# naver/dust3r

Measured on NVIDIA H100. Metric: image-pairs/sec (512x384, ViT-L/B+DPT), higher is better.
Workload: dtype bf16

## Files before the change

dust3r_b200/_lib_fwd.py:

```python
import ctypes as C

F_BIAS, F_GELU, F_RELU, F_OUT_F32, F_RESID_INPLACE = 1, 2, 4, 8, 16
F_ADD0, F_ADD1, F_OUT2_RELU, F_ROPE, F_OUT2_BF16 = 32, 64, 128, 256, 2048


class Linear(C.Structure):
    _fields_ = [('w', C.c_void_p), ('b', C.c_void_p)]


class Norm(C.Structure):
    _fields_ = [('g', C.c_void_p), ('b', C.c_void_p)]


class EncBlock(C.Structure):
    _fields_ = [('norm1', Norm), ('norm2', Norm), ('qkv', Linear), ('proj', Linear), ('fc1', Linear), ('fc2', Linear)]


class DecBlock(C.Structure):
    _fields_ = [('norm1', Norm), ('norm2', Norm), ('norm3', Norm), ('norm_y', Norm),
                ('qkv', Linear), ('proj', Linear), ('projq', Linear), ('projkv', Linear), ('cproj', Linear),
                ('fc1', Linear), ('fc2', Linear)]


class Fusion(C.Structure):
# ... 27 lines not shown
    lib.d3r_conv3x3_bf16.argtypes = [vp, vp, vp, vp, vp, vp, vp, i32, i32, i32, i32, i32, u32, vp]
    lib.d3r_attention_hd64.restype = C.c_int
    lib.d3r_attention_hd64.argtypes = [vp, i64, vp, i64, vp, i64, vp, i64, i32, i32, i32, i32, f32, vp]
    lib.d3r_conv_transpose_bf16.restype = C.c_int
    lib.d3r_conv_transpose_bf16.argtypes = [vp, vp, vp, vp, i32, i32, i32, i32, i32, i32, vp]
    lib.d3r_conv3x3_head_tail.restype = C.c_int
    lib.d3r_conv3x3_head_tail.argtypes = [vp, vp, vp, vp, vp, vp, vp, i32, i32, i32, i32, i32, f32, f32, vp]
    lib.d3r_layernorm_bf16.restype = C.c_int
    lib.d3r_layernorm_bf16.argtypes = [vp, vp, vp, vp, i32, i32, f32, vp]
    lib.d3r_upsample2x_bf16.restype = C.c_int
    lib.d3r_upsample2x_bf16.argtypes = [vp, vp, i32, i32, i32, i32, i32, i32, vp]
    lib.d3r_im2col_3x3_s2_bf16.restype = C.c_int
    lib.d3r_im2col_3x3_s2_bf16.argtypes = [vp, vp, i32, i32, i32, i32, vp]
    lib.d3r_patch_im2col16.restype = C.c_int
    lib.d3r_patch_im2col16.argtypes = [vp, vp, i32, i32, i32, vp]
    lib.d3r_linear_head_postprocess.restype = C.c_int
    lib.d3r_linear_head_postprocess.argtypes = [vp, vp, vp, i32, i32, i32, i32, i32, i32, f32, f32, vp]
    lib.d3r_set_gemm_impl.restype = None
    lib.d3r_set_gemm_impl.argtypes = [i32]
    lib.d3r_set_gemm_store.restype = None
    lib.d3r_set_gemm_store.argtypes = [i32]
    lib.d3r_set_conv_store.restype = None
    lib.d3r_set_conv_store.argtypes = [i32]
    lib.d3r_set_attention_impl.restype = None
    lib.d3r_set_attention_impl.argtypes = [i32]
    lib.d3r_forward_workspace_bytes.restype = i64
    lib.d3r_forward_workspace_bytes.argtypes = [C.POINTER(Model), i32, i32, i32, i32]
    lib.d3r_forward_pairs.restype = C.c_int
    lib.d3r_forward_pairs.argtypes = [C.POINTER(Model), vp, i32, C.POINTER(i32), C.POINTER(i32), i32, i32, i32,
                                      vp, vp, vp, vp, vp, i64, vp]
    lib.d3r_forward_mixed_workspace_bytes.restype = i64
    lib.d3r_forward_mixed_workspace_bytes.argtypes = [C.POINTER(Model), i32, i32, i32, i32, i32]
    lib.d3r_forward_pairs_mixed.restype = C.c_int
    lib.d3r_forward_pairs_mixed.argtypes = [C.POINTER(Model), vp, i32, i32, vp, i32, i32, i32, vp, vp, vp, vp, vp, i64, vp]
    lib.d3r_encode_workspace_bytes.restype = i64
    lib.d3r_encode_workspace_bytes.argtypes = [C.POINTER(Model), i32, i32, i32]
    lib.d3r_encode_images.restype = C.c_int
    lib.d3r_encode_images.argtypes = [C.POINTER(Model), vp, i32, i32, i32, vp, vp, i64, vp]
    lib.d3r_decode_workspace_bytes.restype = i64
    lib.d3r_decode_workspace_bytes.argtypes = [C.POINTER(Model), i32, i32, i32, i32, i32]
    lib.d3r_decode_pairs.restype = C.c_int
    lib.d3r_decode_pairs.argtypes = [C.POINTER(Model), vp, i32, i32, i32, vp, i32, i32, i32, C.POINTER(i32), C.POINTER(i32), i32,
                                     vp, vp, vp, vp, vp, i64, vp]
    lib.d3r_forward_set_debug.restype = C.c_int
    lib.d3r_forward_set_debug.argtypes = [i32, vp, i64]
    lib.d3r_sizeof_model.restype = C.c_int
# ... 1 lines not shown
```

dust3r_b200/csrc/gemm_host.cu:

```cuda
#include "gemm_wgmma.cuh"
#include "gemm_host.h"
#include "prof.h"

namespace d3r {
namespace gemm {

static int pick_block_n(int N, int mode, uint32_t flags, int conv_m_tiles = 0) {
  if (flags & F_HEAD_FINAL) return 128;
  if (conv_m_tiles > 0) return (N == 256 && (conv_m_tiles + 1) / 2 >= 4 * (num_sms() / 2)) ? 256 : 128;
  if (N % 256 == 0 && pick_epi(mode, flags) != EPI_GENERIC) return 256;
  if (N % 128 == 0) return 128;
  if (N % 64 == 0) return 64;
  return (N > 128) ? 128 : 64;
}

static int g_impl = 2;
static int g_pair_min_kb = 4;
static bool use_pair(int bn, int num_kb) { return bn >= 128 && (g_impl == 1 || (g_impl == 2 && num_kb >= g_pair_min_kb)); }

static int g_store = 1;
static int g_conv_store = 1;

static int grid_for(bool pair, int m_tiles, int n_tiles) {
  if (pair) {
    const int items = ((m_tiles + 1) / 2) * n_tiles;
    const int max_clusters = num_sms() / 2;
    return 2 * (items < max_clusters ? items : max_clusters);
  }
  const int items = m_tiles * n_tiles;
  return items < num_sms() ? items : num_sms();
}

static const char* prof_tag(const Params& p, int bn, bool pair) {
  return (p.mode == 1) ? ((p.flags & F_HEAD_FINAL) ? (pair ? "conv3x3_head_tail_2cta" : "conv3x3_head_tail")
                                                   : (pair ? "conv3x3_wgmma_2cta" : "conv3x3_wgmma"))
                       : (bn == 256 ? (pair ? "gemm_wgmma_2cta_bn256" : "gemm_wgmma_bn256")
                                    : (pair ? "gemm_wgmma_2cta_bn128" : (bn == 128 ? "gemm_wgmma_bn128" : "gemm_wgmma_bn64")));
}

template <int BN, int EPI, bool PAIR, bool TMA_STORE = false>
static int launch(const CUtensorMap& ta, const CUtensorMap& tb, const CUtensorMap& to, const Params& p, int m_tiles, int n_tiles,
                  cudaStream_t st) {
  constexpr int kSmem = Cfg<BN, TMA_STORE>::kSmemBytes;
  static unsigned long long attr_devices = 0;
  if (first_launch_on_this_device(attr_devices))
    D3R_CUDA(cudaFuncSetAttribute(gemm_kernel<BN, EPI, PAIR, TMA_STORE>, cudaFuncAttributeMaxDynamicSharedMemorySize, kSmem));
  const int grid = grid_for(PAIR, m_tiles, n_tiles);
  char detail[96];
  snprintf(detail, sizeof(detail), "M=%d N=%d K=%d flags=0x%x mode=%d epi=%d", p.M, p.N, p.K, (unsigned)p.flags, p.mode, EPI);
  prof::Scope scope(prof_tag(p, BN, PAIR), st, 2.0 * double(p.M) * double(p.N) * double(p.K), 0.0, 1, detail);
  D3R_CUDA(pdl::launch_clustered(gemm_kernel<BN, EPI, PAIR, TMA_STORE>, dim3(grid), dim3(kNumThreads), size_t(kSmem), st, PAIR ? 2 : 1,
                                 ta, tb, to, p));
  D3R_LAUNCH_CHECK();
  return D3R_OK;
}

template <int BN, bool PAIR>
static int launch_conv(const CUtensorMap& ta, const CUtensorMap& tb, const CUtensorMap& to, const ConvMaps& cm, const Params& p,
                       int m_tiles, int n_tiles, cudaStream_t st) {
  constexpr int kSmem = Cfg<BN, true>::kSmemBytes;
  static unsigned long long attr_devices = 0;
  if (first_launch_on_this_device(attr_devices))
    D3R_CUDA(cudaFuncSetAttribute(conv_kernel<BN, PAIR>, cudaFuncAttributeMaxDynamicSharedMemorySize, kSmem));
  const int grid = grid_for(PAIR, m_tiles, n_tiles);
  char detail[96];
  snprintf(detail, sizeof(detail), "M=%d N=%d K=%d flags=0x%x mode=%d epi=%d", p.M, p.N, p.K, (unsigned)p.flags, p.mode, EPI_GENERIC);
  prof::Scope scope(prof_tag(p, BN, PAIR), st, 2.0 * double(p.M) * double(p.N) * double(p.K), 0.0, 1, detail);
  D3R_CUDA(pdl::launch_clustered(conv_kernel<BN, PAIR>, dim3(grid), dim3(kNumThreads), size_t(kSmem), st, PAIR ? 2 : 1, ta, tb, to, cm, p));
  D3R_LAUNCH_CHECK();
  return D3R_OK;
}

template <int BN, bool PAIR>
static int dispatch_epi(int epi, const CUtensorMap& ta, const CUtensorMap& tb, const CUtensorMap* to, const Params& p, int m_tiles,
                        int n_tiles, cudaStream_t st) {
  if constexpr (BN == 256) {
    if (to) {
      switch (epi) {
        case EPI_RESID: return launch<BN, EPI_RESID, PAIR, true>(ta, tb, *to, p, m_tiles, n_tiles, st);
// ... 6 lines not shown
    case EPI_RESID: return launch<BN, EPI_RESID, PAIR>(ta, tb, tb, p, m_tiles, n_tiles, st);
    case EPI_ACT: return launch<BN, EPI_ACT, PAIR>(ta, tb, tb, p, m_tiles, n_tiles, st);
    case EPI_ROPE: return launch<BN, EPI_ROPE, PAIR>(ta, tb, tb, p, m_tiles, n_tiles, st);
  }
  if constexpr (BN == 128) return launch<128, EPI_GENERIC, PAIR>(ta, tb, tb, p, m_tiles, n_tiles, st);
  set_error("no BLOCK_N %d kernel for the generic epilogue", BN);
  return D3R_ERR_INVALID;
}

static int dispatch(int bn, const CUtensorMap& ta, const CUtensorMap& tb, const CUtensorMap* to, const Params& p, int m_tiles,
                    cudaStream_t st) {
  const int n_tiles = (p.N + bn - 1) / bn;
  const int epi = (bn >= 128) ? pick_epi(p.mode, p.flags) : EPI_GENERIC;
  const bool pair = use_pair(bn, p.num_kb);
  switch (bn) {
    case 256: return pair ? dispatch_epi<256, true>(epi, ta, tb, to, p, m_tiles, n_tiles, st) : dispatch_epi<256, false>(epi, ta, tb, to, p, m_tiles, n_tiles, st);
    case 128: return pair ? dispatch_epi<128, true>(epi, ta, tb, nullptr, p, m_tiles, n_tiles, st) : dispatch_epi<128, false>(epi, ta, tb, nullptr, p, m_tiles, n_tiles, st);
    case 64: return launch<64, EPI_GENERIC, false>(ta, tb, tb, p, m_tiles, n_tiles, st);
  }
  set_error("unsupported BLOCK_N %d", bn);
  return D3R_ERR_INVALID;
}

static int make_tmap_b(CUtensorMap* m, const void* B, int N, int taps, int Kc, int bn, int num_kb, const char* op) {
  cuuint64_t dims[3] = {(cuuint64_t)Kc, (cuuint64_t)taps, (cuuint64_t)N};
  cuuint64_t str[2] = {(cuuint64_t)Kc * 2, (cuuint64_t)taps * Kc * 2};
  cuuint32_t box[3] = {(cuuint32_t)BLOCK_K, 1, (cuuint32_t)(use_pair(bn, num_kb) ? bn / 2 : bn)};
  return encode_tensor_map(m, B, 3, dims, str, box, op);
}

int gemm_bf16(const void* A, long long lda, const void* B, Params p, cudaStream_t st) {
  D3R_CHECK_ARG(A && B, "gemm: null operand");
  D3R_CHECK_ARG(p.M > 0 && p.N > 0 && p.K > 0, "gemm: bad shape %d %d %d", p.M, p.N, p.K);
  D3R_CHECK_ARG(p.N % 32 == 0, "gemm: N=%d must be a multiple of 32", p.N);
  D3R_CHECK_ARG(p.K % 8 == 0 && lda % 8 == 0, "gemm: K=%d / lda=%lld must be multiples of 8 (16-byte TMA strides)", p.K, lda);
  D3R_CHECK_ARG((reinterpret_cast<uintptr_t>(A) & 15) == 0 && (reinterpret_cast<uintptr_t>(B) & 15) == 0, "gemm: operands must be 16-byte aligned");
  p.mode = 0;
  p.num_kb = (p.K + BLOCK_K - 1) / BLOCK_K;
  const int bn = pick_block_n(p.N, p.mode, p.flags);
  CUtensorMap ta, tb;
  {
    cuuint64_t dims[2] = {(cuuint64_t)p.K, (cuuint64_t)p.M};
    cuuint64_t str[1] = {(cuuint64_t)lda * 2};
    cuuint32_t box[2] = {(cuuint32_t)BLOCK_K, (cuuint32_t)BLOCK_M};
    int rc = encode_tensor_map(&ta, A, 2, dims, str, box, "gemm");
    if (rc) return rc;
  }
  int rc = make_tmap_b(&tb, B, p.N, 1, p.K, bn, p.num_kb, "gemm");
  if (rc) return rc;
  CUtensorMap to;
  const bool f32 = (p.flags & F_RESID_INPLACE) != 0;
  const long long row_bytes = p.ldo * (f32 ? 4 : 2);
  const bool staged = g_store == 1 && bn == 256 && pick_epi(p.mode, p.flags) != EPI_GENERIC && p.ldo >= p.N && row_bytes % 16 == 0 &&
                      (reinterpret_cast<uintptr_t>(p.out) & 15) == 0;
  if (staged) {
    cuuint64_t dims[2] = {(cuuint64_t)p.N, (cuuint64_t)p.M};
    cuuint64_t str[1] = {(cuuint64_t)row_bytes};
    cuuint32_t box[2] = {(cuuint32_t)(f32 ? 32 : 64), 64};
    rc = encode_tensor_map(&to, p.out, 2, dims, str, box, "gemm output", f32 ? CU_TENSOR_MAP_DATA_TYPE_FLOAT32 : CU_TENSOR_MAP_DATA_TYPE_BFLOAT16);
    if (rc) return rc;
  }
  return dispatch(bn, ta, tb, staged ? &to : nullptr, p, (p.M + BLOCK_M - 1) / BLOCK_M, st);
}

static int make_tmap_conv_io(CUtensorMap* m, const void* base, int B, int H, int W, int C, int tile_w, const char* op) {
  const int bw = tile_w < 64 ? tile_w : 64;
  cuuint64_t dims[4] = {(cuuint64_t)C, (cuuint64_t)W, (cuuint64_t)H, (cuuint64_t)B};
  cuuint64_t str[3] = {(cuuint64_t)C * 2, (cuuint64_t)W * C * 2, (cuuint64_t)H * W * C * 2};
  cuuint32_t box[4] = {64, (cuuint32_t)bw, (cuuint32_t)(64 / bw), 1};
  return encode_tensor_map(m, base, 4, dims, str, box, op);
}

static bool aligned16(const void* ptr) { return (reinterpret_cast<uintptr_t>(ptr) & 15) == 0; }

int conv3x3_bf16(const void* x_nhwc, const void* w_packed, int B, int H, int W, int Cin, int Cout, Params p, cudaStream_t st) {
  D3R_CHECK_ARG(x_nhwc && w_packed, "conv3x3: null operand");
  D3R_CHECK_ARG(Cin % 8 == 0 && Cout % 32 == 0, "conv3x3: Cin=%d must be a multiple of 8 and Cout=%d of 32", Cin, Cout);
  p.mode = 1;
  p.M = B * H * W;
  p.N = Cout;
  p.cin_blocks = (Cin + BLOCK_K - 1) / BLOCK_K;
  p.K = 9 * Cin;
  p.num_kb = 9 * p.cin_blocks;
  p.cB = B; p.cH = H; p.cW = W;
  int tw = 16;
  while (tw < W && tw < 128) tw *= 2;
  p.tile_w = tw;
  p.tile_h = BLOCK_M / tw;
  p.tiles_x = (W + p.tile_w - 1) / p.tile_w;
  p.tiles_y = (H + p.tile_h - 1) / p.tile_h;
  p.ldo = Cout;
  const int m_tiles = B * p.tiles_x * p.tiles_y;
  const bool staged = g_conv_store == 1 && (Cout == 256 || Cout == 128) && (p.flags & ~EpiMask<EPI_CONV>::value) == 0 &&
                      aligned16(p.out) && (!(p.flags & F_OUT2_RELU) || aligned16(p.out2)) && (!(p.flags & F_ADD0) || aligned16(p.add0)) &&
                      (!(p.flags & F_ADD1) || aligned16(p.add1));
  const int bn = pick_block_n(p.N, p.mode, p.flags, staged ? m_tiles : 0);
  CUtensorMap ta, tb;
  {
    cuuint64_t dims[4] = {(cuuint64_t)Cin, (cuuint64_t)W, (cuuint64_t)H, (cuuint64_t)B};
    cuuint64_t str[3] = {(cuuint64_t)Cin * 2, (cuuint64_t)W * Cin * 2, (cuuint64_t)H * W * Cin * 2};
    cuuint32_t box[4] = {(cuuint32_t)BLOCK_K, (cuuint32_t)p.tile_w, (cuuint32_t)p.tile_h, 1};
    int rc = encode_tensor_map(&ta, x_nhwc, 4, dims, str, box, "conv3x3");
    if (rc) return rc;
  }
  int rc = make_tmap_b(&tb, w_packed, Cout, 9, Cin, bn, p.num_kb, "conv3x3");
  if (rc) return rc;
  if (!staged) return dispatch(bn, ta, tb, nullptr, p, m_tiles, st);
  CUtensorMap to;
  ConvMaps cm;
  rc = make_tmap_conv_io(&to, p.out, B, H, W, Cout, p.tile_w, "conv3x3 output");
  if (rc) return rc;
  cm.out2 = cm.add0 = cm.add1 = to;
  const struct { uint32_t flag; const void* base; CUtensorMap* map; const char* op; } io[3] = {
      {F_OUT2_RELU, p.out2, &cm.out2, "conv3x3 out2"}, {F_ADD0, p.add0, &cm.add0, "conv3x3 add0"}, {F_ADD1, p.add1, &cm.add1, "conv3x3 add1"}};
  for (const auto& t : io) {
    if (!(p.flags & t.flag)) continue;
    rc = make_tmap_conv_io(t.map, t.base, B, H, W, Cout, p.tile_w, t.op);
    if (rc) return rc;
  }
  const int n_tiles = Cout / bn;
  const bool pair = use_pair(bn, p.num_kb);
  if (bn == 256) return pair ? launch_conv<256, true>(ta, tb, to, cm, p, m_tiles, n_tiles, st) : launch_conv<256, false>(ta, tb, to, cm, p, m_tiles, n_tiles, st);
  return pair ? launch_conv<128, true>(ta, tb, to, cm, p, m_tiles, n_tiles, st) : launch_conv<128, false>(ta, tb, to, cm, p, m_tiles, n_tiles, st);
}

int conv_transpose_bf16(const void* x_nhwc, const void* w_packed, void* out, const float* bias, int B, int h, int w, int Cin, int Cout,
                        int k, cudaStream_t st) {
  D3R_CHECK_ARG(x_nhwc && w_packed && out, "conv_transpose: null buffer");
// ... 16 lines not shown
  D3R_CHECK_ARG(B > 0 && H > 0 && W > 0, "conv3x3_head_tail: bad shape B=%d H=%d W=%d", B, H, W);
  D3R_CHECK_ARG(depth_mode >= 0 && depth_mode <= 2, "conv3x3_head_tail: depth_mode %d out of range", depth_mode);
  D3R_CHECK_ARG(conf_mode >= 0 && conf_mode <= 2, "conv3x3_head_tail: conf_mode %d out of range", conf_mode);
  D3R_CHECK_ARG(conf_mode == 0 || conf, "conv3x3_head_tail: conf_mode %d without a conf buffer", conf_mode);
  Params p{};
  p.flags = F_HEAD_FINAL | (bias ? F_BIAS : 0);
  p.bias = bias;
  p.w4 = w4; p.b4 = b4;
  p.pts3d = pts3d; p.conf = conf;
  p.depth_mode = depth_mode; p.conf_mode = conf_mode;
  p.conf_min = conf_min; p.conf_max = conf_max;
  return conv3x3_bf16(x_nhwc, w_packed, B, H, W, 128, 128, p, st);
}

}
}

using namespace d3r;

extern "C" void d3r_set_gemm_impl(int32_t impl) { gemm::g_impl = impl; }
extern "C" void d3r_set_gemm_pair_min_kblocks(int32_t kb) { gemm::g_pair_min_kb = kb; }
extern "C" void d3r_set_gemm_store(int32_t store) { gemm::g_store = store; }
extern "C" void d3r_set_conv_store(int32_t store) { gemm::g_conv_store = store; }

extern "C" int d3r_gemm_bf16(const void* A, const void* B, void* out, const float* bias, const void* add0, void* out2,
                             int32_t M, int32_t N, int32_t K, int64_t ldo, uint32_t flags, const float* rope_cos,
                             const float* rope_sin, int32_t rope_cols, int32_t tokens_per_img, int32_t grid_w, void* stream) {
  gemm::Params p{};
  p.M = M; p.N = N; p.K = K;
  p.flags = flags;
  p.out = out; p.out2 = out2; p.add0 = add0; p.bias = bias; p.ldo = ldo;
  p.rope_cos = rope_cos; p.rope_sin = rope_sin; p.rope_cols = rope_cols; p.tokens_per_img = tokens_per_img; p.grid_w = grid_w;
  D3R_CHECK_ARG(!(flags & gemm::F_BIAS) || bias, "gemm: F_BIAS without bias");
  D3R_CHECK_ARG(!(flags & gemm::F_ROPE) || (rope_cos && rope_sin && tokens_per_img > 0 && grid_w > 0), "gemm: F_ROPE without tables");
  D3R_CHECK_ARG(!(flags & (gemm::F_CONVT | gemm::F_HEAD_FINAL)),
                "gemm: F_CONVT / F_HEAD_FINAL have their own entry points, d3r_conv_transpose_bf16 / d3r_conv3x3_head_tail");
  return gemm::gemm_bf16(A, K, B, p, (cudaStream_t)stream);
}

extern "C" int d3r_conv3x3_bf16(const void* x_nhwc, const void* w_packed, void* out, const float* bias, const void* add0,
                                const void* add1, void* out2, int32_t B, int32_t H, int32_t W, int32_t Cin, int32_t Cout,
                                uint32_t flags, void* stream) {
  gemm::Params p{};
  p.flags = flags;
  p.out = out; p.out2 = out2; p.add0 = add0; p.add1 = add1; p.bias = bias;
  D3R_CHECK_ARG(!(flags & (gemm::F_CONVT | gemm::F_HEAD_FINAL | gemm::F_ROPE)), "conv3x3: unsupported flag");
// ... 15 lines not shown
```

dust3r_b200/csrc/gemm_wgmma.cuh:

```cuda
#pragma once
#include "d3r_common.cuh"
#include "sm90_ptx.cuh"
#include "pdl.cuh"

namespace d3r {
namespace gemm {

constexpr int BLOCK_M = 128;
constexpr int BLOCK_K = 64;
constexpr int WGMMA_K = 16;
constexpr int kNumThreads = 384;
constexpr int kConsumerWarps = 8;

enum : uint32_t {
  F_BIAS = 1u << 0,
  F_GELU = 1u << 1,
  F_RELU = 1u << 2,
  F_OUT_F32 = 1u << 3,
  F_RESID_INPLACE = 1u << 4,
  F_ADD0 = 1u << 5,
  F_ADD1 = 1u << 6,
  F_OUT2_RELU = 1u << 7,
  F_ROPE = 1u << 8,
  F_CONVT = 1u << 9,
  F_HEAD_FINAL = 1u << 10,
  F_OUT2_BF16 = 1u << 11,
// ... 23 lines not shown
  int conf_mode;
  float conf_min, conf_max;
};

enum : int { EPI_GENERIC = 0, EPI_RESID = 1, EPI_ACT = 2, EPI_ROPE = 3, EPI_CONV = 4 };
template <int EPI> struct EpiMask { static constexpr uint32_t value = 0xFFFFFFFFu; };
template <> struct EpiMask<EPI_RESID> { static constexpr uint32_t value = F_BIAS | F_RESID_INPLACE; };
template <> struct EpiMask<EPI_ACT> { static constexpr uint32_t value = F_BIAS | F_GELU | F_RELU; };
template <> struct EpiMask<EPI_ROPE> { static constexpr uint32_t value = F_BIAS | F_ROPE; };
template <> struct EpiMask<EPI_CONV> { static constexpr uint32_t value = F_BIAS | F_RELU | F_ADD0 | F_ADD1 | F_OUT2_RELU; };

struct ConvMaps {
  CUtensorMap out2, add0, add1;
};

__host__ __device__ inline int pick_epi(int mode, uint32_t flags) {
  if (mode != 0) return EPI_GENERIC;
  if ((flags & ~F_BIAS) == F_RESID_INPLACE) return EPI_RESID;
  if ((flags & ~EpiMask<EPI_ACT>::value) == 0) return EPI_ACT;
  if ((flags & ~EpiMask<EPI_ROPE>::value) == 0) return EPI_ROPE;
  return EPI_GENERIC;
}

template <int BLOCK_N, bool TMA_STORE = false>
struct Cfg {
  static constexpr int kStageA = BLOCK_M * BLOCK_K * 2;
  static constexpr int kStageB = BLOCK_N * BLOCK_K * 2;
  static constexpr int kStages = (BLOCK_N == 256) ? 4 : (BLOCK_N == 128) ? 6 : 8;
  static constexpr int kRing = kStages * (kStageA + kStageB);
  static constexpr int kOutBuf = 64 * 128;
  static constexpr int kStaging = TMA_STORE ? 2 * 2 * kOutBuf : 0;
  static constexpr int kSmemBytes = kRing + kStaging + 1024  + 256  + (TMA_STORE ? 0 : (4 * 128 + 16) * 4) ;
  static_assert(kSmemBytes <= 227 * 1024, "shared memory of one CTA");
};

__device__ __forceinline__ float gelu_erf(float x) {
  constexpr float kU = 0.84932180028801904f;
  constexpr float kP = 0.3275911f * 0.70710678118654752f / kU;
  const float u = fabsf(x) * kU;
  const float t = ptx::rcp_approx(fmaf(kP, u, 1.f));
  float poly = fmaf(0.5f * 1.061405429f, t, 0.5f * -1.453152027f);
  poly = fmaf(poly, t, 0.5f * 1.421413741f);
  poly = fmaf(poly, t, 0.5f * -0.284496736f);
  poly = fmaf(poly, t, 0.5f * 0.254829592f);
  const float e = ptx::ex2_approx(-u * u);
  const float h = x * (poly * t * e);
  return fmaxf(x, 0.f) - fabsf(h);
}

template <int BLOCK_N, int EPI, bool PAIR, bool TMA_STORE>
__device__ __forceinline__ void gemm_body(const CUtensorMap& tmap_a, const CUtensorMap& tmap_b, const CUtensorMap& tmap_o,
                                          const ConvMaps* cm, const Params& p) {
  static_assert(EPI == EPI_CONV ? (TMA_STORE && (BLOCK_N == 256 || BLOCK_N == 128))
                                : (!TMA_STORE || (BLOCK_N == 256 && EPI != EPI_GENERIC)),
                "TMA-store epilogue: specialised projection epilogues on 128x256 tiles, the conv epilogue on 128x256 / 128x128");
  using C = Cfg<BLOCK_N, TMA_STORE>;
  extern __shared__ uint8_t smem_raw[];
  uint8_t* smem = reinterpret_cast<uint8_t*>((reinterpret_cast<uintptr_t>(smem_raw) + 1023) & ~uintptr_t(1023));
  uint8_t* smem_a = smem;
  uint8_t* smem_b = smem + C::kStages * C::kStageA;
  uint8_t* smem_o = smem + C::kRing;
  uint64_t* bars = reinterpret_cast<uint64_t*>(smem + C::kRing + C::kStaging);
  uint64_t* full_bar = bars;
  uint64_t* empty_bar = bars + C::kStages;
  uint64_t* add_bar = bars + 2 * C::kStages;
  float* s_w4 = reinterpret_cast<float*>(reinterpret_cast<uint8_t*>(bars) + 256);

  const int warp = threadIdx.x >> 5, lane = threadIdx.x & 31;
  const uint32_t rank = PAIR ? ptx::cluster_ctarank() : 0u;
  const int n_tiles = (p.N + BLOCK_N - 1) / BLOCK_N;
  const int m_tiles = (p.mode == 1) ? p.cB * p.tiles_y * p.tiles_x : (p.M + BLOCK_M - 1) / BLOCK_M;
  const int m_groups = PAIR ? (m_tiles + 1) / 2 : m_tiles;
  const int total_items = m_groups * n_tiles;
  const int first_item = PAIR ? blockIdx.x / 2 : blockIdx.x;
  const int item_stride = PAIR ? gridDim.x / 2 : gridDim.x;

  if (threadIdx.x == 0) {
    ptx::prefetch_tmap(&tmap_a);
    ptx::prefetch_tmap(&tmap_b);
    if constexpr (TMA_STORE) ptx::prefetch_tmap(&tmap_o);
    for (int s = 0; s < C::kStages; ++s) {
      ptx::mbar_init(ptx::smem_u32(&full_bar[s]), 1);
      ptx::mbar_init(ptx::smem_u32(&empty_bar[s]), (PAIR ? 2 : 1) * kConsumerWarps);
    }
    if constexpr (EPI == EPI_CONV) {
      ptx::prefetch_tmap(&cm->out2);
      ptx::prefetch_tmap(&cm->add0);
      ptx::prefetch_tmap(&cm->add1);
      ptx::mbar_init(ptx::smem_u32(&add_bar[0]), 1);
      ptx::mbar_init(ptx::smem_u32(&add_bar[1]), 1);
    }
    ptx::fence_barrier_init();
  }
  if (!TMA_STORE && (p.flags & F_HEAD_FINAL) && threadIdx.x >= 128) {
    for (int i = threadIdx.x - 128; i < 4 * 128 + 4; i += 256) s_w4[i] = (i < 512) ? p.w4[i] : p.b4[i - 512];
  }
  __syncthreads();
  if constexpr (PAIR) ptx::cluster_sync();
  pdl::sync_with_predecessor();

  if (warp < 4) {
    ptx::setmaxnreg_dec<40>();
    if (warp == 0 && ptx::elect_one()) {
      int stage = 0;
      uint32_t phase = 0;
      for (int item = first_item; item < total_items; item += item_stride) {
        const int tn = item % n_tiles, tm = (item / n_tiles) * (PAIR ? 2 : 1) + int(rank);
        int cb = 0, cy0 = 0, cx0 = 0;
        if (p.mode == 1) {
          cb = tm / (p.tiles_y * p.tiles_x);
          const int r = tm - cb * (p.tiles_y * p.tiles_x);
          cy0 = (r / p.tiles_x) * p.tile_h;
          cx0 = (r % p.tiles_x) * p.tile_w;
        }
        for (int kb = 0; kb < p.num_kb; ++kb) {
          ptx::mbar_wait(ptx::smem_u32(&empty_bar[stage]), phase ^ 1);
          const uint32_t fb = ptx::smem_u32(&full_bar[stage]);
          ptx::mbar_arrive_expect_tx(fb, C::kStageA + C::kStageB);
          const uint32_t sa = ptx::smem_u32(smem_a + stage * C::kStageA);
          const uint32_t sb = ptx::smem_u32(smem_b + stage * C::kStageB);
          int ka, kt = 0;
          if (p.mode == 1) {
            const int tap = kb / p.cin_blocks, cblk = kb - tap * p.cin_blocks;
            const int dy = tap / 3, dx = tap - dy * 3;
            ptx::tma_load_4d(sa, &tmap_a, fb, cblk * BLOCK_K, cx0 + dx - 1, cy0 + dy - 1, cb);
            ka = cblk * BLOCK_K;
            kt = tap;
          } else {
            ptx::tma_load_2d(sa, &tmap_a, fb, kb * BLOCK_K, tm * BLOCK_M);
            ka = kb * BLOCK_K;
          }
          if constexpr (PAIR) {
            constexpr int kHalf = BLOCK_N / 2;
            ptx::tma_load_3d_mc(sb + rank * (kHalf * BLOCK_K * 2), &tmap_b, fb, ka, kt, tn * BLOCK_N + int(rank) * kHalf, 0x3);
          } else {
            ptx::tma_load_3d(sb, &tmap_b, fb, ka, kt, tn * BLOCK_N);
          }
          if (++stage == C::kStages) { stage = 0; phase ^= 1; }
        }
      }
    }
  } else {
    ptx::setmaxnreg_inc<232>();
    const int wg = (threadIdx.x >> 7) - 1;
    const int wq = warp & 3;
    const int q = lane & 3;
    const uint32_t flags = p.flags & EpiMask<EPI>::value;
    constexpr int kNB = BLOCK_N / 8;
    float acc[BLOCK_N / 2];
    int stage = 0;
    uint32_t phase = 0;
    uint32_t out_chunk = 0;
    auto release = [&](int s) {
      if (lane == 0) {
        if constexpr (PAIR) {
          ptx::mbar_arrive_cluster(ptx::smem_u32(&empty_bar[s]), 0);
          ptx::mbar_arrive_cluster(ptx::smem_u32(&empty_bar[s]), 1);
        } else {
          ptx::mbar_arrive(ptx::smem_u32(&empty_bar[s]));
        }
      }
    };
    const bool conv_issuer = EPI == EPI_CONV && (threadIdx.x & 127) == 0;
    const bool conv_two = EPI == EPI_CONV && (flags & (F_OUT2_RELU | F_ADD1)) != 0;
    const bool conv_add = EPI == EPI_CONV && (flags & (F_ADD0 | F_ADD1)) != 0;
    uint32_t add_phase = 0;
    auto conv_box = [&](int tm, int& bx, int& by, int& bb) {
      bb = tm / (p.tiles_y * p.tiles_x);
      const int r = tm - bb * (p.tiles_y * p.tiles_x);
      bx = (r % p.tiles_x) * p.tile_w + (64 * wg) % p.tile_w;
      by = (r / p.tiles_x) * p.tile_h + (64 * wg) / p.tile_w;
    };
    auto out_buf = [&](int i) { return ptx::smem_u32(smem_o + (wg * 2 + i) * C::kOutBuf); };
    auto issue_addends = [&](int tm, int ch) {
      int bx, by, bb;
      conv_box(tm, bx, by, bb);
      const uint32_t b0 = conv_two ? out_buf(0) : out_buf(out_chunk & 1);
      if (conv_two) ptx::bulk_wait_group_read<0>();
      else ptx::bulk_wait_group_read<1>();
      const uint32_t bar = ptx::smem_u32(&add_bar[wg]);
      ptx::mbar_arrive_expect_tx(bar, uint32_t(C::kOutBuf) * (((flags & F_ADD0) ? 1u : 0u) + ((flags & F_ADD1) ? 1u : 0u)));
      if (flags & F_ADD0) ptx::tma_load_4d(b0, &cm->add0, bar, ch, bx, by, bb);
      if (flags & F_ADD1) ptx::tma_load_4d(out_buf(1), &cm->add1, bar, ch, bx, by, bb);
    };
    for (int item = first_item; item < total_items; item += item_stride) {
      const int tn = item % n_tiles, tm = (item / n_tiles) * (PAIR ? 2 : 1) + int(rank);
      if constexpr (EPI == EPI_CONV) {
        if (conv_add && conv_issuer) issue_addends(tm, tn * BLOCK_N);
      }
      int prev = -1;
      for (int kb = 0; kb < p.num_kb; ++kb) {
        ptx::mbar_wait(ptx::smem_u32(&full_bar[stage]), phase);
        const uint64_t da = ptx::desc_kmajor_sw128(ptx::smem_u32(smem_a + stage * C::kStageA + wg * 64 * 128));
        const uint64_t db = ptx::desc_kmajor_sw128(ptx::smem_u32(smem_b + stage * C::kStageB));
        ptx::wgmma_fence();
#pragma unroll
        for (int k = 0; k < BLOCK_K / WGMMA_K; ++k) {
          if constexpr (BLOCK_N == 256) ptx::wgmma_m64n256k16_ss(acc, da + uint64_t(2 * k), db + uint64_t(2 * k), (kb | k) != 0 ? 1u : 0u);
          else if constexpr (BLOCK_N == 128) ptx::wgmma_m64n128k16_ss(acc, da + uint64_t(2 * k), db + uint64_t(2 * k), (kb | k) != 0 ? 1u : 0u);
          else ptx::wgmma_m64n64k16_ss(acc, da + uint64_t(2 * k), db + uint64_t(2 * k), (kb | k) != 0 ? 1u : 0u);
        }
        ptx::wgmma_commit();
        ptx::wgmma_wait<1>();
        if (prev >= 0) release(prev);
        prev = stage;
        if (++stage == C::kStages) { stage = 0; phase ^= 1; }
      }
      ptx::wgmma_wait<0>();
      ptx::reg_fence(acc);
      release(prev);

      bool valid[2];
      long long row_off[2];
      int tok[2] = {0, 0};
      long long pix[2] = {0, 0};
      int ct_b[2] = {0, 0}, ct_iy[2] = {0, 0}, ct_ix[2] = {0, 0};
#pragma unroll
      for (int h = 0; h < 2; ++h) {
        const int row_in_tile = wg * 64 + wq * 16 + (lane >> 2) + 8 * h;
        if (p.mode == 1) {
          const int cb = tm / (p.tiles_y * p.tiles_x);
          const int r = tm - cb * (p.tiles_y * p.tiles_x);
          const int y = (r / p.tiles_x) * p.tile_h + row_in_tile / p.tile_w;
          const int x = (r % p.tiles_x) * p.tile_w + row_in_tile % p.tile_w;
          valid[h] = (tm < m_tiles) && (y < p.cH) && (x < p.cW);
          pix[h] = (long long)(cb * p.cH + y) * p.cW + x;
          row_off[h] = pix[h] * p.ldo;
        } else {
          const int row = tm * BLOCK_M + row_in_tile;
          valid[h] = row < p.M;
          row_off[h] = (long long)row * p.ldo;
          if (flags & F_ROPE) tok[h] = row % p.tokens_per_img;
          if (flags & F_CONVT) {
            ct_b[h] = row / (p.th_in * p.tw_in);
            const int r = row - ct_b[h] * (p.th_in * p.tw_in);
            ct_iy[h] = r / p.tw_in;
            ct_ix[h] = r - ct_iy[h] * p.tw_in;
          }
        }
      }
      if (flags & (F_BIAS | F_GELU)) {
#pragma unroll
        for (int j = 0; j < kNB; ++j) {
          const int c = tn * BLOCK_N + 8 * j + 2 * q;
          float2 b = make_float2(0.f, 0.f);
          if ((flags & F_BIAS) && c < p.N) {
            if (flags & F_CONVT) b = make_float2(__ldg(p.bias + c % p.tCout), __ldg(p.bias + (c + 1) % p.tCout));
            else b = __ldg(reinterpret_cast<const float2*>(p.bias + c));
          }
#pragma unroll
          for (int h = 0; h < 2; ++h) {
            float& v0 = acc[4 * j + 2 * h];
// ... 82 lines not shown
        constexpr int kChunkNB = kChunkCols / 8;
        const bool issuer = (threadIdx.x & 127) == 0;
        const uint32_t sw = lane >> 2;
#pragma unroll
        for (int c = 0; c < BLOCK_N / kChunkCols; ++c) {
          const uint32_t buf = ptx::smem_u32(smem_o + (wg * 2 + (out_chunk & 1)) * C::kOutBuf);
#pragma unroll
          for (int j = 0; j < kChunkNB; ++j)
#pragma unroll
            for (int h = 0; h < 2; ++h) {
              const uint32_t row = wq * 16 + (lane >> 2) + 8 * h;
              float v0 = acc[4 * (c * kChunkNB + j) + 2 * h], v1 = acc[4 * (c * kChunkNB + j) + 2 * h + 1];
              if (flags & F_RELU) { v0 = fmaxf(v0, 0.f); v1 = fmaxf(v1, 0.f); }
              if constexpr (kF32) {
                ptx::st_shared_v2_f32(buf + row * 128 + (((2 * j + (q >> 1)) ^ sw) << 4) + (q & 1) * 8, v0, v1);
              } else {
                ptx::st_shared_b32(buf + row * 128 + ((j ^ sw) << 4) + q * 4, pack_bf16x2(v0, v1));
              }
            }
          ptx::fence_proxy_async();
          if (issuer) ptx::bulk_wait_group_read<0>();
          ptx::named_bar_sync(1 + wg, 128);
          if (issuer) {
            const int c0 = tn * BLOCK_N + c * kChunkCols, r0 = tm * BLOCK_M + wg * 64;
            if constexpr (kF32) ptx::tma_reduce_add_2d(&tmap_o, buf, c0, r0);
            else ptx::tma_store_2d(&tmap_o, buf, c0, r0);
            ptx::bulk_commit_group();
          }
          ++out_chunk;
        }
        continue;
      }
      if (flags & F_HEAD_FINAL) {
        float head_acc[2][4] = {{0.f, 0.f, 0.f, 0.f}, {0.f, 0.f, 0.f, 0.f}};
#pragma unroll
        for (int j = 0; j < kNB; ++j)
#pragma unroll
          for (int h = 0; h < 2; ++h)
#pragma unroll
            for (int e = 0; e < 2; ++e) {
              const float r = fmaxf(acc[4 * j + 2 * h + e], 0.f);
              const int c = 8 * j + 2 * q + e;
#pragma unroll
              for (int o = 0; o < 4; ++o) head_acc[h][o] += r * s_w4[o * 128 + c];
            }
#pragma unroll
        for (int h = 0; h < 2; ++h)
// ... 36 lines not shown
            v0 += a.x; v1 += a.y;
          }
          if (flags & F_RELU) { v0 = fmaxf(v0, 0.f); v1 = fmaxf(v1, 0.f); }
          if (flags & (F_OUT_F32 | F_RESID_INPLACE)) {
            float2* o = reinterpret_cast<float2*>(reinterpret_cast<float*>(p.out) + off);
            if (flags & F_RESID_INPLACE) {
              const float2 r = *o;
              v0 += r.x; v1 += r.y;
            }
            *o = make_float2(v0, v1);
            if (flags & F_OUT2_BF16) *reinterpret_cast<uint32_t*>(reinterpret_cast<__nv_bfloat16*>(p.out2) + off) = pack_bf16x2(v0, v1);
          } else {
            *reinterpret_cast<uint32_t*>(reinterpret_cast<__nv_bfloat16*>(p.out) + off) = pack_bf16x2(v0, v1);
            if (flags & F_OUT2_RELU)
              *reinterpret_cast<uint32_t*>(reinterpret_cast<__nv_bfloat16*>(p.out2) + off) = pack_bf16x2(fmaxf(v0, 0.f), fmaxf(v1, 0.f));
          }
        }
      }
    }
    if constexpr (TMA_STORE) {
      if ((threadIdx.x & 127) == 0) ptx::bulk_wait_group<0>();
    }
  }
  if constexpr (PAIR) ptx::cluster_sync();
}

template <int BLOCK_N, int EPI, bool PAIR, bool TMA_STORE>
__global__ void __launch_bounds__(kNumThreads, 1)
gemm_kernel(const __grid_constant__ CUtensorMap tmap_a, const __grid_constant__ CUtensorMap tmap_b,
            const __grid_constant__ CUtensorMap tmap_o, const Params p) {
  gemm_body<BLOCK_N, EPI, PAIR, TMA_STORE>(tmap_a, tmap_b, tmap_o, nullptr, p);
}

template <int BLOCK_N, bool PAIR>
__global__ void __launch_bounds__(kNumThreads, 1)
conv_kernel(const __grid_constant__ CUtensorMap tmap_a, const __grid_constant__ CUtensorMap tmap_b,
            const __grid_constant__ CUtensorMap tmap_o, const __grid_constant__ ConvMaps cm, const Params p) {
  gemm_body<BLOCK_N, EPI_CONV, PAIR, true>(tmap_a, tmap_b, tmap_o, &cm, p);
}

}
}
```

include/dust3r_b200.h:

```cpp
#ifndef DUST3R_B200_H_
#define DUST3R_B200_H_

#include <stddef.h>
#include <stdint.h>

#ifdef __cplusplus
extern "C" {
#endif

#define D3R_OK 0
#define D3R_ERR_INVALID (-1)
#define D3R_ERR_CUDA (-2)
#define D3R_ERR_UNSUPPORTED_DEVICE (-3)

const char* d3r_last_error(void);
int d3r_abi_version(void);
int d3r_check_device(void);

long long d3r_launch_count(void);
void d3r_launch_count_reset(void);
void d3r_prof_enable(int on);
int d3r_prof_report(char* buf, int cap);
int d3r_prof_dump(char* buf, int cap);

// ... 121 lines not shown
                            int32_t h, int32_t w, int32_t Cin, int32_t Cout, int32_t k, void* stream);

int d3r_conv3x3_head_tail(const void* x_nhwc_dev, const void* w_packed_dev, const float* bias_dev, const float* w4_dev,
                          const float* b4_dev, float* pts3d_dev, float* conf_dev, int32_t B, int32_t H, int32_t W, int32_t depth_mode,
                          int32_t conf_mode, float conf_min, float conf_max, void* stream);

int d3r_layernorm_bf16(const float* x_dev, const float* g_dev, const float* b_dev, void* out_dev, int32_t M, int32_t C, float eps,
                       void* stream);

int d3r_upsample2x_bf16(const void* x_dev, void* out_dev, int32_t B, int32_t H, int32_t W, int32_t C, int32_t Ho, int32_t Wo,
                        void* stream);

int d3r_im2col_3x3_s2_bf16(const void* x_dev, void* out_dev, int32_t B, int32_t H, int32_t W, int32_t C, void* stream);

int d3r_patch_im2col16(const float* img_dev, void* out_dev, int32_t B, int32_t H, int32_t W, void* stream);

int d3r_linear_head_postprocess(const float* feat_dev, float* pts3d_dev, float* conf_dev, int32_t B, int32_t gh, int32_t gw,
                                int32_t nch, int32_t depth_mode, int32_t conf_mode, float conf_min, float conf_max, void* stream);

void d3r_set_gemm_impl(int32_t impl);
void d3r_set_gemm_pair_min_kblocks(int32_t kblocks);
void d3r_set_gemm_store(int32_t store);
void d3r_set_conv_store(int32_t store);

void d3r_set_attention_impl(int32_t impl);

int d3r_clean_pointcloud(int32_t n_imgs, const int32_t* hw_dev, const int64_t* off_dev, int32_t max_area, const float* pts3d_dev,
                         float* conf_dev, const float* depth_dev, const float* K_dev, const float* cams_dev, float tol,
                         float bad_conf, void* stream);
int d3r_procrustes_moments(int32_t n_problems, int32_t n_points, const float* x_dev, const float* y_dev, const float* w_dev,
                           double* out_dev, void* stream);
int d3r_weiszfeld_focal(int32_t n_maps, int32_t H, int32_t W, const float* pts3d_dev, const float* pp_dev, int32_t steps,
                        float* focal_dev, void* stream);
int d3r_nearest_neighbours(int32_t n_queries, int32_t n_points, const float* queries_dev, const float* points_dev, int32_t* nn_dev,
                           void* stream);
int d3r_image_resize_crop_normalize(const uint8_t* src_dev, int32_t H0, int32_t W0, int32_t H1, int32_t W1,
                                    const int32_t* xbounds_dev, const int32_t* xcoefs_dev, int32_t kx,
                                    const int32_t* ybounds_dev, const int32_t* ycoefs_dev, int32_t ky, int32_t row0, int32_t rows,
                                    int32_t crop_x0, int32_t crop_y0, int32_t H2, int32_t W2, const float* lut_dev, uint8_t* tmp_dev,
                                    float* out_dev, void* stream);
int64_t d3r_segment_sky_workspace_bytes(int32_t n_imgs, int64_t total_px);
int d3r_segment_sky(int32_t n_imgs, const int32_t* hw_dev, const int64_t* off_dev, int32_t max_area, int64_t total_px,
                    const uint8_t* rgb_dev, uint8_t* sky_out_dev, void* workspace_dev, int64_t workspace_bytes, void* stream);

typedef struct d3r_linear { const void* w; const float* b; } d3r_linear;
typedef struct d3r_norm { const float* g; const float* b; } d3r_norm;
// ... 82 lines not shown
```

Baseline: 231.9.

## Add ping-pong warpgroup GEMM schedule for residual projections

Adds a ping-pong GEMM kernel in which the two consumer warpgroups each own a 64x256 tile and take turns on the mainloop, handing off through turn barriers. One warpgroup's epilogue then overlaps the other's MMA. B tiles are multicast across a 2-CTA cluster. By default it is enabled only for staged residual-epilogue GEMMs with K up to 1024, which targets the epilogue bubble in the fc2/proj layers. In exchange the M tiles are smaller and the A operand is reloaded more often, and the new barrier and ring-cursor logic adds complexity.

```diff
diff --git a/dust3r_b200/_lib_fwd.py b/dust3r_b200/_lib_fwd.py
--- a/dust3r_b200/_lib_fwd.py
+++ b/dust3r_b200/_lib_fwd.py
@@ -73,6 +73,8 @@
     lib.d3r_set_gemm_store.argtypes = [i32]
     lib.d3r_set_conv_store.restype = None
     lib.d3r_set_conv_store.argtypes = [i32]
+    lib.d3r_set_gemm_schedule.restype = None
+    lib.d3r_set_gemm_schedule.argtypes = [i32]
     lib.d3r_set_attention_impl.restype = None
     lib.d3r_set_attention_impl.argtypes = [i32]
     lib.d3r_forward_workspace_bytes.restype = i64
diff --git a/dust3r_b200/csrc/gemm_host.cu b/dust3r_b200/csrc/gemm_host.cu
--- a/dust3r_b200/csrc/gemm_host.cu
+++ b/dust3r_b200/csrc/gemm_host.cu
@@ -20,6 +20,13 @@
 
 static int g_store = 1;
 static int g_conv_store = 1;
+static int g_schedule = 2;
+constexpr int kPPCluster = 2;
+
+static bool use_pingpong(bool staged, int epi, int num_kb) {
+  if (!staged || g_impl != 2 || !use_pair(256, num_kb)) return false;
+  return g_schedule == 1 || (g_schedule == 2 && epi == EPI_RESID && num_kb <= 1024 / BLOCK_K);
+}
 
 static int grid_for(bool pair, int m_tiles, int n_tiles) {
   if (pair) {
@@ -55,6 +62,52 @@
   return D3R_OK;
 }
 
+template <int EPI, int CL>
+static int pp_max_clusters(int smem) {
+  static int cached[64] = {};
+  int dev = 0;
+  cudaGetDevice(&dev);
+  int& n = cached[dev & 63];
+  if (n > 0) return n;
+  cudaLaunchConfig_t cfg = {};
+  cfg.gridDim = dim3(CL);
+  cfg.blockDim = dim3(kNumThreads);
+  cfg.dynamicSmemBytes = size_t(smem);
+  cudaLaunchAttribute at;
+  at.id = cudaLaunchAttributeClusterDimension;
+  at.val.clusterDim.x = CL;
+  at.val.clusterDim.y = 1;
+  at.val.clusterDim.z = 1;
+  cfg.attrs = &at;
+  cfg.numAttrs = 1;
+  int clusters = 0;
+  if (cudaOccupancyMaxActiveClusters(&clusters, gemm_pp_kernel<EPI, CL>, &cfg) != cudaSuccess) clusters = 0;
+  n = clusters;
+  return n;
+}
+
+template <int EPI, int CL>
+static int launch_pp(const CUtensorMap& ta, const CUtensorMap& tb, const CUtensorMap& to, const Params& p, int m_items, int n_tiles,
+                     cudaStream_t st) {
+  constexpr int kSmem = Cfg<256, true, CL>::kSmemBytes;
+  static unsigned long long attr_devices = 0;
+  if (first_launch_on_this_device(attr_devices))
+    D3R_CUDA(cudaFuncSetAttribute(gemm_pp_kernel<EPI, CL>, cudaFuncAttributeMaxDynamicSharedMemorySize, kSmem));
+  const int max_clusters = pp_max_clusters<EPI, CL>(kSmem);
+  if (max_clusters <= 0) {
+    set_error("gemm: no cluster of %d CTAs with %d bytes of shared memory fits on this device", CL, kSmem);
+    return D3R_ERR_CUDA;
+  }
+  const int items = ((m_items + CL - 1) / CL) * n_tiles;
+  const int grid = CL * (items < max_clusters ? items : max_clusters);
+  char detail[96];
+  snprintf(detail, sizeof(detail), "M=%d N=%d K=%d flags=0x%x mode=%d epi=%d", p.M, p.N, p.K, (unsigned)p.flags, p.mode, EPI);
+  prof::Scope scope("gemm_wgmma_pp_bn256", st, 2.0 * double(p.M) * double(p.N) * double(p.K), 0.0, 1, detail);
+  D3R_CUDA(pdl::launch_clustered(gemm_pp_kernel<EPI, CL>, dim3(grid), dim3(kNumThreads), size_t(kSmem), st, CL, ta, tb, to, p));
+  D3R_LAUNCH_CHECK();
+  return D3R_OK;
+}
+
 template <int BN, bool PAIR>
 static int launch_conv(const CUtensorMap& ta, const CUtensorMap& tb, const CUtensorMap& to, const ConvMaps& cm, const Params& p,
                        int m_tiles, int n_tiles, cudaStream_t st) {
@@ -107,10 +160,10 @@
   return D3R_ERR_INVALID;
 }
 
-static int make_tmap_b(CUtensorMap* m, const void* B, int N, int taps, int Kc, int bn, int num_kb, const char* op) {
+static int make_tmap_b(CUtensorMap* m, const void* B, int N, int taps, int Kc, int box_n, const char* op) {
   cuuint64_t dims[3] = {(cuuint64_t)Kc, (cuuint64_t)taps, (cuuint64_t)N};
   cuuint64_t str[2] = {(cuuint64_t)Kc * 2, (cuuint64_t)taps * Kc * 2};
-  cuuint32_t box[3] = {(cuuint32_t)BLOCK_K, 1, (cuuint32_t)(use_pair(bn, num_kb) ? bn / 2 : bn)};
+  cuuint32_t box[3] = {(cuuint32_t)BLOCK_K, 1, (cuuint32_t)box_n};
   return encode_tensor_map(m, B, 3, dims, str, box, op);
 }
 
@@ -123,27 +176,37 @@
   p.mode = 0;
   p.num_kb = (p.K + BLOCK_K - 1) / BLOCK_K;
   const int bn = pick_block_n(p.N, p.mode, p.flags);
+  const bool f32 = (p.flags & F_RESID_INPLACE) != 0;
+  const long long row_bytes = p.ldo * (f32 ? 4 : 2);
+  const int epi = pick_epi(p.mode, p.flags);
+  const bool staged = g_store == 1 && bn == 256 && epi != EPI_GENERIC && p.ldo >= p.N && row_bytes % 16 == 0 &&
+                      (reinterpret_cast<uintptr_t>(p.out) & 15) == 0;
+  const bool pp = use_pingpong(staged, epi, p.num_kb);
   CUtensorMap ta, tb;
   {
     cuuint64_t dims[2] = {(cuuint64_t)p.K, (cuuint64_t)p.M};
     cuuint64_t str[1] = {(cuuint64_t)lda * 2};
-    cuuint32_t box[2] = {(cuuint32_t)BLOCK_K, (cuuint32_t)BLOCK_M};
+    cuuint32_t box[2] = {(cuuint32_t)BLOCK_K, (cuuint32_t)(pp ? 64 : BLOCK_M)};
     int rc = encode_tensor_map(&ta, A, 2, dims, str, box, "gemm");
     if (rc) return rc;
   }
-  int rc = make_tmap_b(&tb, B, p.N, 1, p.K, bn, p.num_kb, "gemm");
+  int rc = make_tmap_b(&tb, B, p.N, 1, p.K, pp ? bn / kPPCluster : use_pair(bn, p.num_kb) ? bn / 2 : bn, "gemm");
   if (rc) return rc;
   CUtensorMap to;
-  const bool f32 = (p.flags & F_RESID_INPLACE) != 0;
-  const long long row_bytes = p.ldo * (f32 ? 4 : 2);
-  const bool staged = g_store == 1 && bn == 256 && pick_epi(p.mode, p.flags) != EPI_GENERIC && p.ldo >= p.N && row_bytes % 16 == 0 &&
-                      (reinterpret_cast<uintptr_t>(p.out) & 15) == 0;
   if (staged) {
     cuuint64_t dims[2] = {(cuuint64_t)p.N, (cuuint64_t)p.M};
     cuuint64_t str[1] = {(cuuint64_t)row_bytes};
     cuuint32_t box[2] = {(cuuint32_t)(f32 ? 32 : 64), 64};
     rc = encode_tensor_map(&to, p.out, 2, dims, str, box, "gemm output", f32 ? CU_TENSOR_MAP_DATA_TYPE_FLOAT32 : CU_TENSOR_MAP_DATA_TYPE_BFLOAT16);
     if (rc) return rc;
+  }
+  if (pp) {
+    const int m_items = (p.M + 63) / 64, n_tiles = p.N / 256;
+    switch (epi) {
+      case EPI_RESID: return launch_pp<EPI_RESID, kPPCluster>(ta, tb, to, p, m_items, n_tiles, st);
+      case EPI_ACT: return launch_pp<EPI_ACT, kPPCluster>(ta, tb, to, p, m_items, n_tiles, st);
+      case EPI_ROPE: return launch_pp<EPI_ROPE, kPPCluster>(ta, tb, to, p, m_items, n_tiles, st);
+    }
   }
   return dispatch(bn, ta, tb, staged ? &to : nullptr, p, (p.M + BLOCK_M - 1) / BLOCK_M, st);
 }
@@ -188,7 +251,7 @@
     int rc = encode_tensor_map(&ta, x_nhwc, 4, dims, str, box, "conv3x3");
     if (rc) return rc;
   }
-  int rc = make_tmap_b(&tb, w_packed, Cout, 9, Cin, bn, p.num_kb, "conv3x3");
+  int rc = make_tmap_b(&tb, w_packed, Cout, 9, Cin, use_pair(bn, p.num_kb) ? bn / 2 : bn, "conv3x3");
   if (rc) return rc;
   if (!staged) return dispatch(bn, ta, tb, nullptr, p, m_tiles, st);
   CUtensorMap to;
@@ -251,6 +314,7 @@
 extern "C" void d3r_set_gemm_pair_min_kblocks(int32_t kb) { gemm::g_pair_min_kb = kb; }
 extern "C" void d3r_set_gemm_store(int32_t store) { gemm::g_store = store; }
 extern "C" void d3r_set_conv_store(int32_t store) { gemm::g_conv_store = store; }
+extern "C" void d3r_set_gemm_schedule(int32_t schedule) { gemm::g_schedule = schedule; }
 
 extern "C" int d3r_gemm_bf16(const void* A, const void* B, void* out, const float* bias, const void* add0, void* out2,
                              int32_t M, int32_t N, int32_t K, int64_t ldo, uint32_t flags, const float* rope_cos,
diff --git a/dust3r_b200/csrc/gemm_pingpong.h b/dust3r_b200/csrc/gemm_pingpong.h
--- /dev/null
+++ b/dust3r_b200/csrc/gemm_pingpong.h
@@ -0,0 +1,38 @@
+#pragma once
+#include <cstdint>
+
+namespace d3r {
+namespace gemm {
+
+#if defined(__CUDACC__)
+#define D3R_PP_HD __host__ __device__ __forceinline__
+#else
+#define D3R_PP_HD inline
+#endif
+
+struct RingCursor {
+  int slot;
+  uint32_t parity;
+};
+
+D3R_PP_HD void ring_advance(RingCursor& c, int n, int stages) {
+  const int s = c.slot + n;
+  c.parity ^= uint32_t(s / stages) & 1u;
+  c.slot = s % stages;
+}
+
+D3R_PP_HD RingCursor pp_consumer_start(int wg, int num_kb, int stages) {
+  RingCursor c{0, 0u};
+  if (wg == 1) ring_advance(c, num_kb, stages);
+  return c;
+}
+
+D3R_PP_HD int pp_turn_wait_parity(int wg, int t) {
+  if (wg == 0) return t == 0 ? -1 : int((t - 1) & 1);
+  return int(t & 1);
+}
+
+#undef D3R_PP_HD
+
+}
+}
diff --git a/dust3r_b200/csrc/gemm_wgmma.cuh b/dust3r_b200/csrc/gemm_wgmma.cuh
--- a/dust3r_b200/csrc/gemm_wgmma.cuh
+++ b/dust3r_b200/csrc/gemm_wgmma.cuh
@@ -2,6 +2,7 @@
 #include "d3r_common.cuh"
 #include "sm90_ptx.cuh"
 #include "pdl.cuh"
+#include "gemm_pingpong.h"
 
 namespace d3r {
 namespace gemm {
@@ -71,9 +72,10 @@
   return EPI_GENERIC;
 }
 
-template <int BLOCK_N, bool TMA_STORE = false>
+template <int BLOCK_N, bool TMA_STORE = false, int PP = 0>
 struct Cfg {
-  static constexpr int kStageA = BLOCK_M * BLOCK_K * 2;
+  static constexpr int kRowsA = PP ? 64 : BLOCK_M;
+  static constexpr int kStageA = kRowsA * BLOCK_K * 2;
   static constexpr int kStageB = BLOCK_N * BLOCK_K * 2;
   static constexpr int kStages = (BLOCK_N == 256) ? 4 : (BLOCK_N == 128) ? 6 : 8;
   static constexpr int kRing = kStages * (kStageA + kStageB);
@@ -97,13 +99,15 @@
   return fmaxf(x, 0.f) - fabsf(h);
 }
 
-template <int BLOCK_N, int EPI, bool PAIR, bool TMA_STORE>
+template <int BLOCK_N, int EPI, bool PAIR, bool TMA_STORE, int PP = 0>
 __device__ __forceinline__ void gemm_body(const CUtensorMap& tmap_a, const CUtensorMap& tmap_b, const CUtensorMap& tmap_o,
                                           const ConvMaps* cm, const Params& p) {
   static_assert(EPI == EPI_CONV ? (TMA_STORE && (BLOCK_N == 256 || BLOCK_N == 128))
                                 : (!TMA_STORE || (BLOCK_N == 256 && EPI != EPI_GENERIC)),
                 "TMA-store epilogue: specialised projection epilogues on 128x256 tiles, the conv epilogue on 128x256 / 128x128");
-  using C = Cfg<BLOCK_N, TMA_STORE>;
+  static_assert(!PP || (TMA_STORE && !PAIR && EPI != EPI_CONV), "ping-pong: the specialised projection epilogues only");
+  using C = Cfg<BLOCK_N, TMA_STORE, PP>;
+  constexpr int kCluster = PP ? PP : PAIR ? 2 : 1;
   extern __shared__ uint8_t smem_raw[];
   uint8_t* smem = reinterpret_cast<uint8_t*>((reinterpret_cast<uintptr_t>(smem_raw) + 1023) & ~uintptr_t(1023));
   uint8_t* smem_a = smem;
@@ -113,16 +117,17 @@
   uint64_t* full_bar = bars;
   uint64_t* empty_bar = bars + C::kStages;
   uint64_t* add_bar = bars + 2 * C::kStages;
+  uint64_t* turn_bar = bars + 2 * C::kStages + 2;
   float* s_w4 = reinterpret_cast<float*>(reinterpret_cast<uint8_t*>(bars) + 256);
 
   const int warp = threadIdx.x >> 5, lane = threadIdx.x & 31;
-  const uint32_t rank = PAIR ? ptx::cluster_ctarank() : 0u;
+  const uint32_t rank = kCluster > 1 ? ptx::cluster_ctarank() : 0u;
   const int n_tiles = (p.N + BLOCK_N - 1) / BLOCK_N;
-  const int m_tiles = (p.mode == 1) ? p.cB * p.tiles_y * p.tiles_x : (p.M + BLOCK_M - 1) / BLOCK_M;
-  const int m_groups = PAIR ? (m_tiles + 1) / 2 : m_tiles;
+  const int m_tiles = (p.mode == 1) ? p.cB * p.tiles_y * p.tiles_x : (p.M + C::kRowsA - 1) / C::kRowsA;
+  const int m_groups = (m_tiles + kCluster - 1) / kCluster;
   const int total_items = m_groups * n_tiles;
-  const int first_item = PAIR ? blockIdx.x / 2 : blockIdx.x;
-  const int item_stride = PAIR ? gridDim.x / 2 : gridDim.x;
+  const int first_item = blockIdx.x / kCluster;
+  const int item_stride = gridDim.x / kCluster;
 
   if (threadIdx.x == 0) {
     ptx::prefetch_tmap(&tmap_a);
@@ -130,7 +135,11 @@
     if constexpr (TMA_STORE) ptx::prefetch_tmap(&tmap_o);
     for (int s = 0; s < C::kStages; ++s) {
       ptx::mbar_init(ptx::smem_u32(&full_bar[s]), 1);
-      ptx::mbar_init(ptx::smem_u32(&empty_bar[s]), (PAIR ? 2 : 1) * kConsumerWarps);
+      ptx::mbar_init(ptx::smem_u32(&empty_bar[s]), PP ? PP * (kConsumerWarps / 2) : (PAIR ? 2 : 1) * kConsumerWarps);
+    }
+    if constexpr (PP) {
+      ptx::mbar_init(ptx::smem_u32(&turn_bar[0]), 1);
+      ptx::mbar_init(ptx::smem_u32(&turn_bar[1]), 1);
     }
     if constexpr (EPI == EPI_CONV) {
       ptx::prefetch_tmap(&cm->out2);
@@ -145,7 +154,7 @@
     for (int i = threadIdx.x - 128; i < 4 * 128 + 4; i += 256) s_w4[i] = (i < 512) ? p.w4[i] : p.b4[i - 512];
   }
   __syncthreads();
-  if constexpr (PAIR) ptx::cluster_sync();
+  if constexpr (kCluster > 1) ptx::cluster_sync();
   pdl::sync_with_predecessor();
 
   if (warp < 4) {
@@ -154,7 +163,7 @@
       int stage = 0;
       uint32_t phase = 0;
       for (int item = first_item; item < total_items; item += item_stride) {
-        const int tn = item % n_tiles, tm = (item / n_tiles) * (PAIR ? 2 : 1) + int(rank);
+        const int tn = item % n_tiles, tm = (item / n_tiles) * kCluster + int(rank);
         int cb = 0, cy0 = 0, cx0 = 0;
         if (p.mode == 1) {
           cb = tm / (p.tiles_y * p.tiles_x);
@@ -176,10 +185,13 @@
             ka = cblk * BLOCK_K;
             kt = tap;
           } else {
-            ptx::tma_load_2d(sa, &tmap_a, fb, kb * BLOCK_K, tm * BLOCK_M);
+            ptx::tma_load_2d(sa, &tmap_a, fb, kb * BLOCK_K, tm * C::kRowsA);
             ka = kb * BLOCK_K;
           }
-          if constexpr (PAIR) {
+          if constexpr (PP) {
+            constexpr int kPart = BLOCK_N / PP;
+            ptx::tma_load_3d_mc(sb + rank * (kPart * BLOCK_K * 2), &tmap_b, fb, ka, kt, tn * BLOCK_N + int(rank) * kPart, uint16_t((1u << PP) - 1));
+          } else if constexpr (PAIR) {
             constexpr int kHalf = BLOCK_N / 2;
             ptx::tma_load_3d_mc(sb + rank * (kHalf * BLOCK_K * 2), &tmap_b, fb, ka, kt, tn * BLOCK_N + int(rank) * kHalf, 0x3);
           } else {
@@ -200,9 +212,17 @@
     int stage = 0;
     uint32_t phase = 0;
     uint32_t out_chunk = 0;
+    if constexpr (PP) {
+      const RingCursor c0 = pp_consumer_start(wg, p.num_kb, C::kStages);
+      stage = c0.slot;
+      phase = c0.parity;
+    }
     auto release = [&](int s) {
       if (lane == 0) {
-        if constexpr (PAIR) {
+        if constexpr (PP) {
+#pragma unroll
+          for (uint32_t r = 0; r < uint32_t(PP); ++r) ptx::mbar_arrive_cluster(ptx::smem_u32(&empty_bar[s]), r);
+        } else if constexpr (PAIR) {
           ptx::mbar_arrive_cluster(ptx::smem_u32(&empty_bar[s]), 0);
           ptx::mbar_arrive_cluster(ptx::smem_u32(&empty_bar[s]), 1);
         } else {
@@ -232,15 +252,21 @@
       if (flags & F_ADD0) ptx::tma_load_4d(b0, &cm->add0, bar, ch, bx, by, bb);
       if (flags & F_ADD1) ptx::tma_load_4d(out_buf(1), &cm->add1, bar, ch, bx, by, bb);
     };
-    for (int item = first_item; item < total_items; item += item_stride) {
-      const int tn = item % n_tiles, tm = (item / n_tiles) * (PAIR ? 2 : 1) + int(rank);
+    int local = 0;
+    for (int item = first_item; item < total_items; item += item_stride, ++local) {
+      const int tn = item % n_tiles, tm = (item / n_tiles) * kCluster + int(rank);
+      if constexpr (PP) {
+        if ((local & 1) != wg) continue;
+        const int tp = pp_turn_wait_parity(wg, local >> 1);
+        if (tp >= 0) ptx::mbar_wait(ptx::smem_u32(&turn_bar[wg]), uint32_t(tp));
+      }
       if constexpr (EPI == EPI_CONV) {
         if (conv_add && conv_issuer) issue_addends(tm, tn * BLOCK_N);
       }
       int prev = -1;
       for (int kb = 0; kb < p.num_kb; ++kb) {
         ptx::mbar_wait(ptx::smem_u32(&full_bar[stage]), phase);
-        const uint64_t da = ptx::desc_kmajor_sw128(ptx::smem_u32(smem_a + stage * C::kStageA + wg * 64 * 128));
+        const uint64_t da = ptx::desc_kmajor_sw128(ptx::smem_u32(smem_a + stage * C::kStageA + (PP ? 0 : wg * 64 * 128)));
         const uint64_t db = ptx::desc_kmajor_sw128(ptx::smem_u32(smem_b + stage * C::kStageB));
         ptx::wgmma_fence();
 #pragma unroll
@@ -255,6 +281,13 @@
         prev = stage;
         if (++stage == C::kStages) { stage = 0; phase ^= 1; }
       }
+      if constexpr (PP) {
+        if ((threadIdx.x & 127) == 0) ptx::mbar_arrive(ptx::smem_u32(&turn_bar[wg ^ 1]));
+        RingCursor c{stage, phase};
+        ring_advance(c, p.num_kb, C::kStages);
+        stage = c.slot;
+        phase = c.parity;
+      }
       ptx::wgmma_wait<0>();
       ptx::reg_fence(acc);
       release(prev);
@@ -266,7 +299,7 @@
       int ct_b[2] = {0, 0}, ct_iy[2] = {0, 0}, ct_ix[2] = {0, 0};
 #pragma unroll
       for (int h = 0; h < 2; ++h) {
-        const int row_in_tile = wg * 64 + wq * 16 + (lane >> 2) + 8 * h;
+        const int row_in_tile = (PP ? 0 : wg * 64) + wq * 16 + (lane >> 2) + 8 * h;
         if (p.mode == 1) {
           const int cb = tm / (p.tiles_y * p.tiles_x);
           const int r = tm - cb * (p.tiles_y * p.tiles_x);
@@ -276,7 +309,7 @@
           pix[h] = (long long)(cb * p.cH + y) * p.cW + x;
           row_off[h] = pix[h] * p.ldo;
         } else {
-          const int row = tm * BLOCK_M + row_in_tile;
+          const int row = tm * C::kRowsA + row_in_tile;
           valid[h] = row < p.M;
           row_off[h] = (long long)row * p.ldo;
           if (flags & F_ROPE) tok[h] = row % p.tokens_per_img;
@@ -405,7 +438,7 @@
           if (issuer) ptx::bulk_wait_group_read<0>();
           ptx::named_bar_sync(1 + wg, 128);
           if (issuer) {
-            const int c0 = tn * BLOCK_N + c * kChunkCols, r0 = tm * BLOCK_M + wg * 64;
+            const int c0 = tn * BLOCK_N + c * kChunkCols, r0 = tm * C::kRowsA + (PP ? 0 : wg * 64);
             if constexpr (kF32) ptx::tma_reduce_add_2d(&tmap_o, buf, c0, r0);
             else ptx::tma_store_2d(&tmap_o, buf, c0, r0);
             ptx::bulk_commit_group();
@@ -488,7 +521,7 @@
       if ((threadIdx.x & 127) == 0) ptx::bulk_wait_group<0>();
     }
   }
-  if constexpr (PAIR) ptx::cluster_sync();
+  if constexpr (kCluster > 1) ptx::cluster_sync();
 }
 
 template <int BLOCK_N, int EPI, bool PAIR, bool TMA_STORE>
@@ -498,6 +531,13 @@
   gemm_body<BLOCK_N, EPI, PAIR, TMA_STORE>(tmap_a, tmap_b, tmap_o, nullptr, p);
 }
 
+template <int EPI, int CLUSTER>
+__global__ void __launch_bounds__(kNumThreads, 1)
+gemm_pp_kernel(const __grid_constant__ CUtensorMap tmap_a, const __grid_constant__ CUtensorMap tmap_b,
+               const __grid_constant__ CUtensorMap tmap_o, const Params p) {
+  gemm_body<256, EPI, false, true, CLUSTER>(tmap_a, tmap_b, tmap_o, nullptr, p);
+}
+
 template <int BLOCK_N, bool PAIR>
 __global__ void __launch_bounds__(kNumThreads, 1)
 conv_kernel(const __grid_constant__ CUtensorMap tmap_a, const __grid_constant__ CUtensorMap tmap_b,
diff --git a/include/dust3r_b200.h b/include/dust3r_b200.h
--- a/include/dust3r_b200.h
+++ b/include/dust3r_b200.h
@@ -167,6 +167,7 @@
 void d3r_set_gemm_pair_min_kblocks(int32_t kblocks);
 void d3r_set_gemm_store(int32_t store);
 void d3r_set_conv_store(int32_t store);
+void d3r_set_gemm_schedule(int32_t schedule);
 
 void d3r_set_attention_impl(int32_t impl);
 
```

After: 232.0 (median of 6 runs). Within noise of the previous version (+0.0%).
